# phymhan/pc-gan

Hardware: AMD Instinct MI355X
Metric: images/sec (G+D step) 128x128 bs32 per GPU (higher is better)
Workload: dtype f32; 1 GPU; wsgan_emb UTKFace-shaped 128x128 bs32/GPU fp32: 9-block ResnetGenerator + 3-layer PatchGAN + ResNet-18 Elo encoder@224 + AlexNet IP@224, full optimize_parameters(); global_batch=32, parallelism=dp1

## Files before the change

pc-gan_amd/csrc/wgrad_rowring.hip:

```cpp
#include "common.h"

namespace pcgan {

typedef _Float16 rr_h8 __attribute__((ext_vector_type(8)));
typedef _Float16 rr_h4 __attribute__((ext_vector_type(4)));
typedef float rr_f16v __attribute__((ext_vector_type(16)));

struct RowRingArgs {
    const float* X;
    const float* DY;
    float* part;
    float* scales;
    const float* x_amax;
    const float* dy_amax;
    int x_namax, dy_namax;
    int N, C, K, H, W;
    int nmt, ncb;
    int strips, strips_per_split, nwg;
};

__global__ void __launch_bounds__(256, 2) rowring_wgrad_kernel(RowRingArgs a) {
    __shared__ __attribute__((aligned(16))) rr_h8 Xs[4 * 3 * 2 * 2 * 32 + 128];
    __shared__ float scratch[16];
    const int tid = threadIdx.x, lane = tid & 63, lo = lane & 31, hi = lane >> 5;
    const int wave = __builtin_amdgcn_readfirstlane(tid >> 6);
    const int wg = ((int)blockIdx.x & 7) * ((int)gridDim.x >> 3) + ((int)blockIdx.x >> 3);
    if (wg >= a.nwg) return;
    const int tiles = a.nmt * a.ncb;
    const int split = wg / tiles, tile = wg - split * tiles;
    const int mt = tile % a.nmt, cb = tile / a.nmt;
    const int H = a.H, W = a.W;

    const float sx = pow2_scale(block_max(thread_max_of_partials(a.x_amax, a.x_namax, tid, 256), scratch));
    __syncthreads();
    const float sdy = pow2_scale(block_max(thread_max_of_partials(a.dy_amax, a.dy_namax, tid, 256), scratch));
    if (wg == 0 && tid == 0) {
        a.scales[0] = sx;
        a.scales[1] = sdy;
    }

    const int ch = tid >> 3, q = tid & 7;
    char* const xs_bytes = reinterpret_cast<char*>(&Xs[0]);
    auto rec_off = [&](int slot, int s, int piece, int khalf, int c) -> unsigned {
        return (unsigned)((((((slot * 3 + s) * 2 + piece) * 2 + khalf) * 32) + c) * 16);
    };

    rr_f16v acc[9];
#pragma unroll
    for (int t = 0; t < 9; ++t)
#pragma unroll
        for (int r = 0; r < 16; ++r) acc[t][r] = 0.f;

    const int wq = W >> 4;
    const int s_begin = split * a.strips_per_split;
    const int s_end = s_begin + a.strips_per_split < a.strips ? s_begin + a.strips_per_split : a.strips;
    const int HW = H * W;
    const __amdgpu_buffer_rsrc_t rX = __builtin_amdgcn_make_buffer_rsrc(const_cast<float*>(a.X), 0, (int)((size_t)a.N * a.C * HW * 4), 0x00020000);
    const __amdgpu_buffer_rsrc_t rD = __builtin_amdgcn_make_buffer_rsrc(const_cast<float*>(a.DY), 0, (int)((size_t)a.N * a.K * HW * 4), 0x00020000);
    typedef unsigned int rr_u4 __attribute__((ext_vector_type(4)));
    const unsigned vod = (unsigned)(((mt * 128 + wave * 32 + lo) * HW + 8 * hi) * 4);
    for (int strip = s_begin; strip < s_end; ++strip) {
        const int n = strip / wq, x0 = (strip - n * wq) << 4;
        const int colq = q == 0 ? (x0 == 0 ? 1 : x0 - 1) : (q >= 5 ? (x0 + 16 >= W ? W - 2 : x0 + 16) : x0 + 4 * (q - 1));
        const int esel = colq & 3;
        const unsigned vox = (unsigned)((ch * HW + (colq & ~3)) * 4);
        const unsigned sox = (unsigned)((n * a.C + cb * 32) * HW * 4);
        const unsigned sod = (unsigned)((n * a.K * HW + x0) * 4);
        auto ldrow = [&](int py) -> rr_u4 {
            int sy = (py > H + 1 ? H + 1 : py) - 1;
            sy = sy < 0 ? -sy : sy;
            sy = sy >= H ? 2 * (H - 1) - sy : sy;
            return __builtin_amdgcn_raw_buffer_load_b128(rX, vox, sox + (unsigned)(sy * W * 4), 0);
        };
        auto lddy = [&](int y, rr_u4& u0, rr_u4& u1) {
            const int yy = y < H ? y : H - 1;
            u0 = __builtin_amdgcn_raw_buffer_load_b128(rD, vod, sod + (unsigned)(yy * W * 4), 0);
            u1 = __builtin_amdgcn_raw_buffer_load_b128(rD, vod + 16u, sod + (unsigned)(yy * W * 4), 0);
        };
        const bool owns = q >= 1 && q <= 4;
        const int jq = q - 1;
        const unsigned wbase = owns ? (unsigned)(((jq >> 1) * 32 + ch) * 16 + (jq & 1) * 8) : (unsigned)(4 * 3 * 2 * 2 * 32 * 16 + tid * 8);
        const unsigned wmul = owns ? 1u : 0u;
        struct RowRegs {
            unsigned H01, H23, L01, L23, left, right;
        };
        auto pk = [](_Float16 lo16, _Float16 hi16) -> unsigned {
            return (unsigned)__builtin_bit_cast(unsigned short, lo16) | ((unsigned)__builtin_bit_cast(unsigned short, hi16) << 16);
        };
        auto split_row = [&](const rr_u4& raw, RowRegs& g) {
            float v[4] = {__uint_as_float(raw[0]), __uint_as_float(raw[1]), __uint_as_float(raw[2]), __uint_as_float(raw[3])};
            const float pick = esel == 0 ? v[0] : (esel == 1 ? v[1] : (esel == 2 ? v[2] : v[3]));
            v[3] = q == 0 ? pick : v[3];
            v[0] = q >= 5 ? pick : v[0];
            _Float16 u0, u1, u2, u3, w0, w1, w2, w3;
            split2h(v[0] * sx, u0, w0);
            split2h(v[1] * sx, u1, w1);
            split2h(v[2] * sx, u2, w2);
            split2h(v[3] * sx, u3, w3);
            g.H01 = pk(u0, u1);
            g.H23 = pk(u2, u3);
            g.L01 = pk(w0, w1);
            g.L23 = pk(w2, w3);
        };
        auto edges = [&](RowRegs& g) {
            const int e3 = (int)((g.H23 >> 16) | (g.L23 & 0xffff0000u));
            const int e0 = (int)((g.H01 & 0xffffu) | (g.L01 << 16));
            g.left = (unsigned)__builtin_amdgcn_update_dpp(0, e3, 0x111, 0xf, 0xf, false);
            g.right = (unsigned)__builtin_amdgcn_update_dpp(0, e0, 0x101, 0xf, 0xf, false);
        };
        typedef unsigned int rr_u2 __attribute__((ext_vector_type(2)));
        auto write_copy = [&](int slot, int sc, const RowRegs& g) {
            rr_u2 Hq, Lq;
            const unsigned Hmid = __builtin_amdgcn_alignbyte(g.H23, g.H01, 2), Lmid = __builtin_amdgcn_alignbyte(g.L23, g.L01, 2);
            if (sc == 0) {
                Hq = rr_u2{(g.left & 0xffffu) | (g.H01 << 16), Hmid};
                Lq = rr_u2{(g.left >> 16) | (g.L01 << 16), Lmid};
            } else if (sc == 1) {
                Hq = rr_u2{g.H01, g.H23};
                Lq = rr_u2{g.L01, g.L23};
            } else {
                Hq = rr_u2{Hmid, (g.H23 >> 16) | (g.right << 16)};
                Lq = rr_u2{Lmid, (g.L23 >> 16) | (g.right & 0xffff0000u)};
            }
            *reinterpret_cast<rr_u2*>(xs_bytes + wbase + wmul * rec_off(slot, sc, 0, 0, 0)) = Hq;
            *reinterpret_cast<rr_u2*>(xs_bytes + wbase + wmul * rec_off(slot, sc, 1, 0, 0)) = Lq;
        };
        auto build = [&](int slot, const rr_u4& raw) {
            RowRegs g;
            split_row(raw, g);
            edges(g);
            write_copy(slot, 0, g);
            write_copy(slot, 1, g);
            write_copy(slot, 2, g);
        };
        rr_h8 Bh[3], Bl[3];
        auto rdB = [&](int buf, int ybase, int tap) {
            const int r = tap / 3, sc = tap % 3;
            Bh[buf] = *reinterpret_cast<const rr_h8*>(xs_bytes + rec_off((ybase + r) & 3, sc, 0, hi, lo));
            Bl[buf] = *reinterpret_cast<const rr_h8*>(xs_bytes + rec_off((ybase + r) & 3, sc, 1, hi, lo));
        };
        struct AFrag {
            rr_h8 h, l;
        };
        auto stage = [&](int y, const AFrag& Acur, AFrag& Anext, const rr_u4& din0, const rr_u4& din1, const rr_u4& xin, rr_u4& dout0, rr_u4& dout1,
                         rr_u4& xout) {
            __builtin_amdgcn_sched_barrier(0);
            lddy(y + 2, dout0, dout1);
            xout = ldrow(y + 4);
            const float dv[8] = {__uint_as_float(din0[0]), __uint_as_float(din0[1]), __uint_as_float(din0[2]), __uint_as_float(din0[3]),
                                 __uint_as_float(din1[0]), __uint_as_float(din1[1]), __uint_as_float(din1[2]), __uint_as_float(din1[3])};
            RowRegs g;
            const int wslot = (y + 3) & 3;
#pragma unroll
            for (int t = 0; t < 9; ++t) {
                __builtin_amdgcn_sched_barrier(0);
                if (t + 2 < 9) rdB((t + 2) % 3, y, t + 2);
                else rdB((t + 2) % 3, y + 1, t + 2 - 9);
                rr_f16v c = acc[t];
                c = __builtin_amdgcn_mfma_f32_32x32x16_f16(Acur.l, Bh[t % 3], c, 0, 0, 0);
                c = __builtin_amdgcn_mfma_f32_32x32x16_f16(Acur.h, Bl[t % 3], c, 0, 0, 0);
                c = __builtin_amdgcn_mfma_f32_32x32x16_f16(Acur.h, Bh[t % 3], c, 0, 0, 0);
                acc[t] = c;
                if (t < 8) {
                    _Float16 u, v;
                    split2h(dv[t] * sdy, u, v);
                    Anext.h[t] = u;
                    Anext.l[t] = v;
                }
                if (t == 0) split_row(xin, g);
                if (t == 1) edges(g);
                if (t == 2) write_copy(wslot, 0, g);
                if (t == 3) write_copy(wslot, 1, g);
                if (t == 4) write_copy(wslot, 2, g);
            }
            __builtin_amdgcn_sched_barrier(0);
            __builtin_amdgcn_s_waitcnt(0xC87F);
            __builtin_amdgcn_s_barrier();
            __builtin_amdgcn_sched_barrier(0);
        };
        rr_u4 r0 = ldrow(0), r1 = ldrow(1), r2 = ldrow(2), xa = ldrow(3), xb2, dA0, dA1, da0, da1, db0, db1;
        lddy(0, dA0, dA1);
        lddy(1, da0, da1);
        __syncthreads();
        build(0, r0);
        build(1, r1);
        build(2, r2);
        AFrag A0, A1;
        {
            const float dv[8] = {__uint_as_float(dA0[0]), __uint_as_float(dA0[1]), __uint_as_float(dA0[2]), __uint_as_float(dA0[3]),
                                 __uint_as_float(dA1[0]), __uint_as_float(dA1[1]), __uint_as_float(dA1[2]), __uint_as_float(dA1[3])};
#pragma unroll
            for (int j = 0; j < 8; ++j) {
                _Float16 u, v;
                split2h(dv[j] * sdy, u, v);
                A0.h[j] = u;
                A0.l[j] = v;
            }
        }
        __syncthreads();
        rdB(0, 0, 0);
        rdB(1, 0, 1);
        int y = 0;
#pragma unroll 1
        for (; y + 1 < H; y += 2) {
            stage(y, A0, A1, da0, da1, xa, db0, db1, xb2);
            stage(y + 1, A1, A0, db0, db1, xb2, da0, da1, xa);
        }
        if (y < H) stage(y, A0, A1, da0, da1, xa, db0, db1, xb2);
    }

#pragma unroll
    for (int t = 0; t < 9; ++t) {
        float* out = a.part + (((size_t)split * 9 + t) * a.K + mt * 128 + wave * 32) * a.C + cb * 32 + lo;
#pragma unroll
        for (int r = 0; r < 16; ++r) out[(size_t)((r >> 2) * 8 + hi * 4 + (r & 3)) * a.C] = acc[t][r];
    }
}

typedef __bf16 rr_b8 __attribute__((ext_vector_type(8)));
typedef unsigned int rr_w4 __attribute__((ext_vector_type(4)));
typedef unsigned int rr_w2 __attribute__((ext_vector_type(2)));

__global__ void __launch_bounds__(256, 2) rowring_wgrad_bf16_kernel(RowRingArgs a) {
    __shared__ __attribute__((aligned(16))) rr_h8 Xs[4 * 3 * 2 * 32 + 128];
    const int tid = threadIdx.x, lane = tid & 63, lo = lane & 31, hi = lane >> 5;
    const int wave = __builtin_amdgcn_readfirstlane(tid >> 6);
    const int wg = ((int)blockIdx.x & 7) * ((int)gridDim.x >> 3) + ((int)blockIdx.x >> 3);
    if (wg >= a.nwg) return;
    const int tiles = a.nmt * a.ncb;
    const int split = wg / tiles, tile = wg - split * tiles;
    const int mt = tile % a.nmt, cb = tile / a.nmt;
    const int H = a.H, W = a.W, HW = H * W;
    if (wg == 0 && tid == 0) {
        a.scales[0] = 1.f;
        a.scales[1] = 1.f;
    }
    const int ch = tid >> 3, q = tid & 7;
    char* const xs_bytes = reinterpret_cast<char*>(&Xs[0]);
    auto rec_off = [&](int slot, int s, int khalf, int c) -> unsigned { return (unsigned)(((((slot * 3 + s) * 2 + khalf) * 32) + c) * 16); };
    rr_f16v acc[9];
#pragma unroll
    for (int t = 0; t < 9; ++t)
#pragma unroll
        for (int r = 0; r < 16; ++r) acc[t][r] = 0.f;
    const int wq = W >> 4;
    const int s_begin = split * a.strips_per_split;
    const int s_end = s_begin + a.strips_per_split < a.strips ? s_begin + a.strips_per_split : a.strips;
    const __amdgpu_buffer_rsrc_t rX = __builtin_amdgcn_make_buffer_rsrc(const_cast<float*>(a.X), 0, (int)((size_t)a.N * a.C * HW * 2), 0x00020000);
    const __amdgpu_buffer_rsrc_t rD = __builtin_amdgcn_make_buffer_rsrc(const_cast<float*>(a.DY), 0, (int)((size_t)a.N * a.K * HW * 2), 0x00020000);
    const unsigned vod = (unsigned)(((mt * 128 + wave * 32 + lo) * HW + 8 * hi) * 2);
    const bool owns = q >= 1 && q <= 4;
    const int jq = q - 1;
    const unsigned wbase = owns ? (unsigned)(((jq >> 1) * 32 + ch) * 16 + (jq & 1) * 8) : (unsigned)(4 * 3 * 2 * 32 * 16 + tid * 8);
    const unsigned wmul = owns ? 1u : 0u;
    for (int strip = s_begin; strip < s_end; ++strip) {
        const int n = strip / wq, x0 = (strip - n * wq) << 4;
        const int colq = q == 0 ? (x0 == 0 ? 1 : x0 - 1) : (q >= 5 ? (x0 + 16 >= W ? W - 2 : x0 + 16) : x0 + 4 * (q - 1));
        const int esel = colq & 3;
        const unsigned vox = (unsigned)((ch * HW + (colq & ~3)) * 2);
        const unsigned sox = (unsigned)((n * a.C + cb * 32) * HW * 2);
        const unsigned sod = (unsigned)((n * a.K * HW + x0) * 2);
        auto ldrow = [&](int py) -> rr_w2 {
            int sy = (py > H + 1 ? H + 1 : py) - 1;
            sy = sy < 0 ? -sy : sy;
            sy = sy >= H ? 2 * (H - 1) - sy : sy;
            return __builtin_amdgcn_raw_buffer_load_b64(rX, vox, sox + (unsigned)(sy * W * 2), 0);
        };
        auto lddy = [&](int y) -> rr_w4 {
            return __builtin_amdgcn_raw_buffer_load_b128(rD, y < H ? vod : 0x80000000u, y < H ? sod + (unsigned)(y * W * 2) : 0u, 0);
        };
        struct RowRegs {
            unsigned E01, E23, left, right;
        };
        auto take_row = [&](const rr_w2& raw, RowRegs& g) {
            const unsigned w = (esel & 2) ? raw[1] : raw[0];
            const unsigned pick = (esel & 1) ? (w >> 16) : (w & 0xffffu);
            g.E01 = q >= 5 ? ((raw[0] & 0xffff0000u) | pick) : raw[0];
            g.E23 = q == 0 ? ((raw[1] & 0xffffu) | (pick << 16)) : raw[1];
        };
        auto edges = [&](RowRegs& g) {
            g.left = (unsigned)__builtin_amdgcn_update_dpp(0, (int)(g.E23 >> 16), 0x111, 0xf, 0xf, false);
            g.right = (unsigned)__builtin_amdgcn_update_dpp(0, (int)(g.E01 & 0xffffu), 0x101, 0xf, 0xf, false);
        };
        auto write_copy = [&](int slot, int sc, const RowRegs& g) {
            const unsigned mid = __builtin_amdgcn_alignbyte(g.E23, g.E01, 2);
            rr_w2 v;
            if (sc == 0) v = rr_w2{g.left | (g.E01 << 16), mid};
            else if (sc == 1) v = rr_w2{g.E01, g.E23};
            else v = rr_w2{mid, (g.E23 >> 16) | (g.right << 16)};
            *reinterpret_cast<rr_w2*>(xs_bytes + wbase + wmul * rec_off(slot, sc, 0, 0)) = v;
        };
        auto build = [&](int slot, const rr_w2& raw) {
            RowRegs g;
            take_row(raw, g);
            edges(g);
            write_copy(slot, 0, g);
            write_copy(slot, 1, g);
            write_copy(slot, 2, g);
        };
        rr_h8 Bq[3];
        auto rdB = [&](int buf, int ybase, int tap) {
            const int r = tap / 3, sc = tap % 3;
            Bq[buf] = *reinterpret_cast<const rr_h8*>(xs_bytes + rec_off((ybase + r) & 3, sc, hi, lo));
        };
        rr_w4 dring[4];
        rr_w2 xring[4];
        const rr_w2 r0 = ldrow(0), r1 = ldrow(1), r2 = ldrow(2);
#pragma unroll
        for (int k = 0; k < 4; ++k) {
            dring[k] = lddy(k);
            xring[k] = ldrow(k + 3);
        }
        __syncthreads();
        build(0, r0);
        build(1, r1);
        build(2, r2);
        __syncthreads();
        rdB(0, 0, 0);
        rdB(1, 0, 1);
#pragma unroll 1
        for (int y0 = 0; y0 < H; y0 += 4) {
#pragma unroll
            for (int k = 0; k < 4; ++k) {
                const int y = y0 + k;
                const rr_b8 A = __builtin_bit_cast(rr_b8, dring[k]);
                RowRegs g;
                const int wslot = (y + 3) & 3;
#pragma unroll
                for (int t = 0; t < 9; ++t) {
                    __builtin_amdgcn_sched_barrier(0);
                    if (t + 2 < 9) rdB((t + 2) % 3, y, t + 2);
                    else rdB((t + 2) % 3, y + 1, t + 2 - 9);
                    acc[t] = __builtin_amdgcn_mfma_f32_32x32x16_bf16(A, __builtin_bit_cast(rr_b8, Bq[t % 3]), acc[t], 0, 0, 0);
                    if (t == 0) take_row(xring[k], g);
                    if (t == 1) edges(g);
                    if (t == 2) write_copy(wslot, 0, g);
                    if (t == 3) write_copy(wslot, 1, g);
                    if (t == 4) write_copy(wslot, 2, g);
                }
                __builtin_amdgcn_sched_barrier(0);
                dring[k] = lddy(y + 4);
                xring[k] = ldrow(y + 7);
                __builtin_amdgcn_s_waitcnt(0xC47F);
                __builtin_amdgcn_s_barrier();
                __builtin_amdgcn_sched_barrier(0);
            }
        }
    }
#pragma unroll
    for (int t = 0; t < 9; ++t) {
        float* out = a.part + (((size_t)split * 9 + t) * a.K + mt * 128 + wave * 32) * a.C + cb * 32 + lo;
#pragma unroll
        for (int r = 0; r < 16; ++r) out[(size_t)((r >> 2) * 8 + hi * 4 + (r & 3)) * a.C] = acc[t][r];
    }
}

struct RowRingPlan {
    int nmt, ncb, strips, per, splits;
    size_t part_bytes, total;
};
static bool rowring_plan(const pcgan_conv_desc* d, RowRingPlan* p) {
    if (!d || (d->dtype != PCGAN_F32 && d->dtype != PCGAN_BF16) || d->R != 3 || d->S != 3 || d->stride != 1 || d->pad != 1 || d->pad_mode != 1 || d->P != d->H || d->Q != d->W)
        return false;
    if (d->H < 3 || d->W < 16 || d->W % 16 != 0 || d->K % 128 != 0 || d->C % 32 != 0 || d->N < 1) return false;
    if ((size_t)d->N * d->C * d->H * d->W * 4 >= 0x80000000ull || (size_t)d->N * d->K * d->H * d->W * 4 >= 0x80000000ull) return false;
    if (d->dtype == PCGAN_BF16 && option(OPT_WGRAD_ROWRING) == 3) return false;
    p->nmt = d->K / 128;
    p->ncb = d->C / 32;
    p->strips = d->N * (d->W / 16);
    const int tiles = p->nmt * p->ncb;
    int cus = 256, dev = 0;
    if (hipGetDevice(&dev) == hipSuccess) (void)hipDeviceGetAttribute(&cus, hipDeviceAttributeMultiprocessorCount, dev);
    if (cus <= 0) cus = 256;
    int want = (2 * cus) / tiles;
    want = want < 1 ? 1 : (want > p->strips ? p->strips : want);
    p->per = (p->strips + want - 1) / want;
    p->splits = (p->strips + p->per - 1) / p->per;
    p->part_bytes = (size_t)p->splits * 9 * d->K * d->C * 4;
    p->total = 256 + align_up(p->part_bytes, 256);
    return true;
}

}

extern "C" int pcgan_conv2d_wgrad_rowring_supported(const pcgan_conv_desc* d) {
    pcgan::RowRingPlan p;
    return pcgan::rowring_plan(d, &p) ? 1 : 0;
}

extern "C" size_t pcgan_conv2d_wgrad_rowring_workspace_bytes(const pcgan_conv_desc* d) {
    pcgan::RowRingPlan p;
    return pcgan::rowring_plan(d, &p) ? p.total : 0;
}

extern "C" int pcgan_conv2d_bwd_weight_rowring(const pcgan_conv_desc* d, const void* x, const float* x_amax, int n_xamax, const void* dy,
                                               const float* dy_amax, int n_dyamax, float* dw, int accumulate, void* ws, size_t ws_bytes,
                                               pcgan_stream_t s) {
    using namespace pcgan;
    RowRingPlan p;
    PCGAN_CHECK(rowring_plan(d, &p), "conv2d_bwd_weight_rowring: unsupported shape (3x3 stride 1 reflection padding 1, fp32, W %% 16 == 0, K %% 128 == 0, C %% 32 == 0)");
    const bool half = d->dtype == PCGAN_BF16;
    PCGAN_CHECK(x && dy && dw && ws && (half || (x_amax && dy_amax && n_xamax > 0 && n_dyamax > 0)), "conv2d_bwd_weight_rowring: null pointer");
    PCGAN_CHECK(ws_bytes >= p.total, "conv2d_bwd_weight_rowring: workspace too small (%zu < %zu)", ws_bytes, p.total);
    hipStream_t st = (hipStream_t)s;
    RowRingArgs a;
    a.X = (const float*)x; a.DY = (const float*)dy;
    a.scales = (float*)ws;
    a.part = (float*)((char*)ws + 256);
    a.x_amax = x_amax; a.dy_amax = dy_amax; a.x_namax = n_xamax; a.dy_namax = n_dyamax;
    a.N = d->N; a.C = d->C; a.K = d->K; a.H = d->H; a.W = d->W;
    a.nmt = p.nmt; a.ncb = p.ncb;
    a.strips = p.strips; a.strips_per_split = p.per;
    a.nwg = p.nmt * p.ncb * p.splits;
    {
        TimerScope whole(timer_kind_res(d, TIMER_RES_WGRAD), st);
        {
            TimerScope main_only(timer_kind_res(d, TIMER_RES_WGRAD_MAIN), st);
            if (half) hipLaunchKernelGGL(rowring_wgrad_bf16_kernel, dim3((unsigned)((a.nwg + 7) / 8 * 8)), dim3(256), 0, st, a);
            else hipLaunchKernelGGL(rowring_wgrad_kernel, dim3((unsigned)((a.nwg + 7) / 8 * 8)), dim3(256), 0, st, a);
        }
        if (launch_wgd_reduce(a.part, dw, a.scales, p.splits, d->K, d->C, accumulate, st)) return 2;
    }
    PCGAN_LAUNCH_CHECK();
    return 0;
}
```

Baseline: 1218 images/sec.

## Pair two strip splits per 512-thread block and reduce partials in LDS

The row-ring weight-gradient kernels now launch 512-thread blocks in which two 256-thread halves each process a separate strip split, each with its own LDS ring. At the end the second half hands its accumulators to the first through LDS in double-buffered steps, so each block writes one summed partial. This halves the partial buffers that go to global memory and that the following reduce kernel must read. In exchange, launch bounds change from 256x2 to 512x1, the two halves synchronise at the end, and a half with fewer strips than its partner runs padded iterations whose dy loads are masked so they contribute nothing.

```diff
diff --git a/pc-gan_amd/csrc/wgrad_rowring.hip b/pc-gan_amd/csrc/wgrad_rowring.hip
--- a/pc-gan_amd/csrc/wgrad_rowring.hip
+++ b/pc-gan_amd/csrc/wgrad_rowring.hip
@@ -17,30 +17,37 @@
     int N, C, K, H, W;
     int nmt, ncb;
     int strips, strips_per_split, nwg;
+    int pair;
 };
 
-__global__ void __launch_bounds__(256, 2) rowring_wgrad_kernel(RowRingArgs a) {
-    __shared__ __attribute__((aligned(16))) rr_h8 Xs[4 * 3 * 2 * 2 * 32 + 128];
+#define RR_HAND_FLOAT4 1024
+
+__global__ void __launch_bounds__(512, 1) rowring_wgrad_kernel(RowRingArgs a) {
+    constexpr int RING = 4 * 3 * 2 * 2 * 32 + 128;
+    __shared__ __attribute__((aligned(16))) rr_h8 Xs[2 * RING];
+    static_assert(2 * RING * 16 >= 2 * RR_HAND_FLOAT4 * 16, "the hand-over buffers live in the ring storage");
     __shared__ float scratch[16];
-    const int tid = threadIdx.x, lane = tid & 63, lo = lane & 31, hi = lane >> 5;
-    const int wave = __builtin_amdgcn_readfirstlane(tid >> 6);
+    const int lane = (int)threadIdx.x & 63, lo = lane & 31, hi = lane >> 5;
+    const int wave8 = __builtin_amdgcn_readfirstlane((int)threadIdx.x >> 6);
+    const int half = wave8 >> 2, wave = wave8 & 3, tid = (int)threadIdx.x & 255;
     const int wg = ((int)blockIdx.x & 7) * ((int)gridDim.x >> 3) + ((int)blockIdx.x >> 3);
     if (wg >= a.nwg) return;
     const int tiles = a.nmt * a.ncb;
-    const int split = wg / tiles, tile = wg - split * tiles;
+    const int pj = wg / tiles, tile = wg - pj * tiles;
+    const int split = pj * a.pair + half;
     const int mt = tile % a.nmt, cb = tile / a.nmt;
     const int H = a.H, W = a.W;
 
-    const float sx = pow2_scale(block_max(thread_max_of_partials(a.x_amax, a.x_namax, tid, 256), scratch));
+    const float sx = pow2_scale(block_max(thread_max_of_partials(a.x_amax, a.x_namax, (int)threadIdx.x, (int)blockDim.x), scratch));
     __syncthreads();
-    const float sdy = pow2_scale(block_max(thread_max_of_partials(a.dy_amax, a.dy_namax, tid, 256), scratch));
-    if (wg == 0 && tid == 0) {
+    const float sdy = pow2_scale(block_max(thread_max_of_partials(a.dy_amax, a.dy_namax, (int)threadIdx.x, (int)blockDim.x), scratch));
+    if (wg == 0 && threadIdx.x == 0) {
         a.scales[0] = sx;
         a.scales[1] = sdy;
     }
 
     const int ch = tid >> 3, q = tid & 7;
-    char* const xs_bytes = reinterpret_cast<char*>(&Xs[0]);
+    char* const xs_bytes = reinterpret_cast<char*>(&Xs[half * RING]);
     auto rec_off = [&](int slot, int s, int piece, int khalf, int c) -> unsigned {
         return (unsigned)((((((slot * 3 + s) * 2 + piece) * 2 + khalf) * 32) + c) * 16);
     };
@@ -54,18 +61,23 @@
     const int wq = W >> 4;
     const int s_begin = split * a.strips_per_split;
     const int s_end = s_begin + a.strips_per_split < a.strips ? s_begin + a.strips_per_split : a.strips;
+    const int sA = pj * a.pair * a.strips_per_split;
+    const int iters = sA + a.strips_per_split < a.strips ? a.strips_per_split : a.strips - sA;
     const int HW = H * W;
     const __amdgpu_buffer_rsrc_t rX = __builtin_amdgcn_make_buffer_rsrc(const_cast<float*>(a.X), 0, (int)((size_t)a.N * a.C * HW * 4), 0x00020000);
     const __amdgpu_buffer_rsrc_t rD = __builtin_amdgcn_make_buffer_rsrc(const_cast<float*>(a.DY), 0, (int)((size_t)a.N * a.K * HW * 4), 0x00020000);
     typedef unsigned int rr_u4 __attribute__((ext_vector_type(4)));
     const unsigned vod = (unsigned)(((mt * 128 + wave * 32 + lo) * HW + 8 * hi) * 4);
-    for (int strip = s_begin; strip < s_end; ++strip) {
+    for (int it = 0; it < iters; ++it) {
+        const bool live = s_begin + it < s_end;
+        const int strip = live ? s_begin + it : a.strips - 1;
         const int n = strip / wq, x0 = (strip - n * wq) << 4;
         const int colq = q == 0 ? (x0 == 0 ? 1 : x0 - 1) : (q >= 5 ? (x0 + 16 >= W ? W - 2 : x0 + 16) : x0 + 4 * (q - 1));
         const int esel = colq & 3;
         const unsigned vox = (unsigned)((ch * HW + (colq & ~3)) * 4);
         const unsigned sox = (unsigned)((n * a.C + cb * 32) * HW * 4);
-        const unsigned sod = (unsigned)((n * a.K * HW + x0) * 4);
+        const unsigned vod_s = live ? vod : 0x80000000u;
+        const unsigned sod = live ? (unsigned)((n * a.K * HW + x0) * 4) : 0u;
         auto ldrow = [&](int py) -> rr_u4 {
             int sy = (py > H + 1 ? H + 1 : py) - 1;
             sy = sy < 0 ? -sy : sy;
@@ -74,12 +86,12 @@
         };
         auto lddy = [&](int y, rr_u4& u0, rr_u4& u1) {
             const int yy = y < H ? y : H - 1;
-            u0 = __builtin_amdgcn_raw_buffer_load_b128(rD, vod, sod + (unsigned)(yy * W * 4), 0);
-            u1 = __builtin_amdgcn_raw_buffer_load_b128(rD, vod + 16u, sod + (unsigned)(yy * W * 4), 0);
+            u0 = __builtin_amdgcn_raw_buffer_load_b128(rD, vod_s, sod + (unsigned)(yy * W * 4), 0);
+            u1 = __builtin_amdgcn_raw_buffer_load_b128(rD, vod_s + 16u, sod + (unsigned)(yy * W * 4), 0);
         };
         const bool owns = q >= 1 && q <= 4;
         const int jq = q - 1;
-        const unsigned wbase = owns ? (unsigned)(((jq >> 1) * 32 + ch) * 16 + (jq & 1) * 8) : (unsigned)(4 * 3 * 2 * 2 * 32 * 16 + tid * 8);
+        const unsigned wbase = owns ? (unsigned)(((jq >> 1) * 32 + ch) * 16 + (jq & 1) * 8) : (unsigned)((RING - 128) * 16 + tid * 8);
         const unsigned wmul = owns ? 1u : 0u;
         struct RowRegs {
             unsigned H01, H23, L01, L23, left, right;
@@ -209,11 +221,38 @@
         if (y < H) stage(y, A0, A1, da0, da1, xa, db0, db1, xb2);
     }
 
-#pragma unroll
-    for (int t = 0; t < 9; ++t) {
-        float* out = a.part + (((size_t)split * 9 + t) * a.K + mt * 128 + wave * 32) * a.C + cb * 32 + lo;
-#pragma unroll
-        for (int r = 0; r < 16; ++r) out[(size_t)((r >> 2) * 8 + hi * 4 + (r & 3)) * a.C] = acc[t][r];
+    auto store_tap = [&](int t, const rr_f16v& v) {
+        float* out = a.part + (((size_t)pj * 9 + t) * a.K + mt * 128 + wave * 32) * a.C + cb * 32 + lo;
+#pragma unroll
+        for (int r = 0; r < 16; ++r) out[(size_t)((r >> 2) * 8 + hi * 4 + (r & 3)) * a.C] = v[r];
+    };
+    if (a.pair == 2) {
+        float4* const hand = reinterpret_cast<float4*>(&Xs[0]);
+        __syncthreads();
+#pragma unroll
+        for (int t = 0; t <= 9; ++t) {
+            if (t < 9 && half == 1) {
+#pragma unroll
+                for (int j = 0; j < 4; ++j)
+                    hand[(t & 1) * RR_HAND_FLOAT4 + j * 256 + tid] = make_float4(acc[t][4 * j], acc[t][4 * j + 1], acc[t][4 * j + 2], acc[t][4 * j + 3]);
+            }
+            if (t > 0 && half == 0) {
+                rr_f16v v = acc[t - 1];
+#pragma unroll
+                for (int j = 0; j < 4; ++j) {
+                    const float4 b = hand[((t - 1) & 1) * RR_HAND_FLOAT4 + j * 256 + tid];
+                    v[4 * j] += b.x;
+                    v[4 * j + 1] += b.y;
+                    v[4 * j + 2] += b.z;
+                    v[4 * j + 3] += b.w;
+                }
+                store_tap(t - 1, v);
+            }
+            if (t < 9) __syncthreads();
+        }
+    } else {
+#pragma unroll
+        for (int t = 0; t < 9; ++t) store_tap(t, acc[t]);
     }
 }
 
@@ -221,22 +260,26 @@
 typedef unsigned int rr_w4 __attribute__((ext_vector_type(4)));
 typedef unsigned int rr_w2 __attribute__((ext_vector_type(2)));
 
-__global__ void __launch_bounds__(256, 2) rowring_wgrad_bf16_kernel(RowRingArgs a) {
-    __shared__ __attribute__((aligned(16))) rr_h8 Xs[4 * 3 * 2 * 32 + 128];
-    const int tid = threadIdx.x, lane = tid & 63, lo = lane & 31, hi = lane >> 5;
-    const int wave = __builtin_amdgcn_readfirstlane(tid >> 6);
+__global__ void __launch_bounds__(512, 1) rowring_wgrad_bf16_kernel(RowRingArgs a) {
+    constexpr int RING = RR_HAND_FLOAT4;
+    static_assert(RING >= 4 * 3 * 2 * 32 + 128, "a half's ring fits its share of the storage");
+    __shared__ __attribute__((aligned(16))) rr_h8 Xs[2 * RING];
+    const int lane = (int)threadIdx.x & 63, lo = lane & 31, hi = lane >> 5;
+    const int wave8 = __builtin_amdgcn_readfirstlane((int)threadIdx.x >> 6);
+    const int half = wave8 >> 2, wave = wave8 & 3, tid = (int)threadIdx.x & 255;
     const int wg = ((int)blockIdx.x & 7) * ((int)gridDim.x >> 3) + ((int)blockIdx.x >> 3);
     if (wg >= a.nwg) return;
     const int tiles = a.nmt * a.ncb;
-    const int split = wg / tiles, tile = wg - split * tiles;
+    const int pj = wg / tiles, tile = wg - pj * tiles;
+    const int split = pj * a.pair + half;
     const int mt = tile % a.nmt, cb = tile / a.nmt;
     const int H = a.H, W = a.W, HW = H * W;
-    if (wg == 0 && tid == 0) {
+    if (wg == 0 && threadIdx.x == 0) {
         a.scales[0] = 1.f;
         a.scales[1] = 1.f;
     }
     const int ch = tid >> 3, q = tid & 7;
-    char* const xs_bytes = reinterpret_cast<char*>(&Xs[0]);
+    char* const xs_bytes = reinterpret_cast<char*>(&Xs[half * RING]);
     auto rec_off = [&](int slot, int s, int khalf, int c) -> unsigned { return (unsigned)(((((slot * 3 + s) * 2 + khalf) * 32) + c) * 16); };
     rr_f16v acc[9];
 #pragma unroll
@@ -246,6 +289,8 @@
     const int wq = W >> 4;
     const int s_begin = split * a.strips_per_split;
     const int s_end = s_begin + a.strips_per_split < a.strips ? s_begin + a.strips_per_split : a.strips;
+    const int sA = pj * a.pair * a.strips_per_split;
+    const int iters = sA + a.strips_per_split < a.strips ? a.strips_per_split : a.strips - sA;
     const __amdgpu_buffer_rsrc_t rX = __builtin_amdgcn_make_buffer_rsrc(const_cast<float*>(a.X), 0, (int)((size_t)a.N * a.C * HW * 2), 0x00020000);
     const __amdgpu_buffer_rsrc_t rD = __builtin_amdgcn_make_buffer_rsrc(const_cast<float*>(a.DY), 0, (int)((size_t)a.N * a.K * HW * 2), 0x00020000);
     const unsigned vod = (unsigned)(((mt * 128 + wave * 32 + lo) * HW + 8 * hi) * 2);
@@ -253,7 +298,9 @@
     const int jq = q - 1;
     const unsigned wbase = owns ? (unsigned)(((jq >> 1) * 32 + ch) * 16 + (jq & 1) * 8) : (unsigned)(4 * 3 * 2 * 32 * 16 + tid * 8);
     const unsigned wmul = owns ? 1u : 0u;
-    for (int strip = s_begin; strip < s_end; ++strip) {
+    for (int it = 0; it < iters; ++it) {
+        const bool live = s_begin + it < s_end;
+        const int strip = live ? s_begin + it : a.strips - 1;
         const int n = strip / wq, x0 = (strip - n * wq) << 4;
         const int colq = q == 0 ? (x0 == 0 ? 1 : x0 - 1) : (q >= 5 ? (x0 + 16 >= W ? W - 2 : x0 + 16) : x0 + 4 * (q - 1));
         const int esel = colq & 3;
@@ -267,7 +314,8 @@
             return __builtin_amdgcn_raw_buffer_load_b64(rX, vox, sox + (unsigned)(sy * W * 2), 0);
         };
         auto lddy = [&](int y) -> rr_w4 {
-            return __builtin_amdgcn_raw_buffer_load_b128(rD, y < H ? vod : 0x80000000u, y < H ? sod + (unsigned)(y * W * 2) : 0u, 0);
+            const bool on = live && y < H;
+            return __builtin_amdgcn_raw_buffer_load_b128(rD, on ? vod : 0x80000000u, on ? sod + (unsigned)(y * W * 2) : 0u, 0);
         };
         struct RowRegs {
             unsigned E01, E23, left, right;
@@ -347,16 +395,44 @@
             }
         }
     }
-#pragma unroll
-    for (int t = 0; t < 9; ++t) {
-        float* out = a.part + (((size_t)split * 9 + t) * a.K + mt * 128 + wave * 32) * a.C + cb * 32 + lo;
-#pragma unroll
-        for (int r = 0; r < 16; ++r) out[(size_t)((r >> 2) * 8 + hi * 4 + (r & 3)) * a.C] = acc[t][r];
+    auto store_tap = [&](int t, const rr_f16v& v) {
+        float* out = a.part + (((size_t)pj * 9 + t) * a.K + mt * 128 + wave * 32) * a.C + cb * 32 + lo;
+#pragma unroll
+        for (int r = 0; r < 16; ++r) out[(size_t)((r >> 2) * 8 + hi * 4 + (r & 3)) * a.C] = v[r];
+    };
+    if (a.pair == 2) {
+        float4* const hand = reinterpret_cast<float4*>(&Xs[0]);
+        __syncthreads();
+#pragma unroll
+        for (int t = 0; t <= 9; ++t) {
+            if (t < 9 && half == 1) {
+#pragma unroll
+                for (int j = 0; j < 4; ++j)
+                    hand[(t & 1) * RR_HAND_FLOAT4 + j * 256 + tid] = make_float4(acc[t][4 * j], acc[t][4 * j + 1], acc[t][4 * j + 2], acc[t][4 * j + 3]);
+            }
+            if (t > 0 && half == 0) {
+                rr_f16v v = acc[t - 1];
+#pragma unroll
+                for (int j = 0; j < 4; ++j) {
+                    const float4 b = hand[((t - 1) & 1) * RR_HAND_FLOAT4 + j * 256 + tid];
+                    v[4 * j] += b.x;
+                    v[4 * j + 1] += b.y;
+                    v[4 * j + 2] += b.z;
+                    v[4 * j + 3] += b.w;
+                }
+                store_tap(t - 1, v);
+            }
+            if (t < 9) __syncthreads();
+        }
+    } else {
+#pragma unroll
+        for (int t = 0; t < 9; ++t) store_tap(t, acc[t]);
     }
 }
 
 struct RowRingPlan {
     int nmt, ncb, strips, per, splits;
+    int pair, nparts;
     size_t part_bytes, total;
 };
 static bool rowring_plan(const pcgan_conv_desc* d, RowRingPlan* p) {
@@ -376,6 +452,8 @@
     want = want < 1 ? 1 : (want > p->strips ? p->strips : want);
     p->per = (p->strips + want - 1) / want;
     p->splits = (p->strips + p->per - 1) / p->per;
+    p->pair = option(OPT_WGRAD_ROWRING) == 4 ? 1 : 2;
+    p->nparts = (p->splits + p->pair - 1) / p->pair;
     p->part_bytes = (size_t)p->splits * 9 * d->K * d->C * 4;
     p->total = 256 + align_up(p->part_bytes, 256);
     return true;
@@ -411,15 +489,16 @@
     a.N = d->N; a.C = d->C; a.K = d->K; a.H = d->H; a.W = d->W;
     a.nmt = p.nmt; a.ncb = p.ncb;
     a.strips = p.strips; a.strips_per_split = p.per;
-    a.nwg = p.nmt * p.ncb * p.splits;
+    a.pair = p.pair;
+    a.nwg = p.nmt * p.ncb * p.nparts;
     {
         TimerScope whole(timer_kind_res(d, TIMER_RES_WGRAD), st);
         {
             TimerScope main_only(timer_kind_res(d, TIMER_RES_WGRAD_MAIN), st);
-            if (half) hipLaunchKernelGGL(rowring_wgrad_bf16_kernel, dim3((unsigned)((a.nwg + 7) / 8 * 8)), dim3(256), 0, st, a);
-            else hipLaunchKernelGGL(rowring_wgrad_kernel, dim3((unsigned)((a.nwg + 7) / 8 * 8)), dim3(256), 0, st, a);
-        }
-        if (launch_wgd_reduce(a.part, dw, a.scales, p.splits, d->K, d->C, accumulate, st)) return 2;
+            if (half) hipLaunchKernelGGL(rowring_wgrad_bf16_kernel, dim3((unsigned)((a.nwg + 7) / 8 * 8)), dim3(256 * p.pair), 0, st, a);
+            else hipLaunchKernelGGL(rowring_wgrad_kernel, dim3((unsigned)((a.nwg + 7) / 8 * 8)), dim3(256 * p.pair), 0, st, a);
+        }
+        if (launch_wgd_reduce(a.part, dw, a.scales, p.nparts, d->K, d->C, accumulate, st)) return 2;
     }
     PCGAN_LAUNCH_CHECK();
     return 0;
```

Result: no change. 1213 images/sec (-0.4%).
